# DoubangoTelecom/compv

Hardware: AMD Instinct MI355X
Metric: Mpixels/s Sobel->Canny->HoughSHT on 4K uint8 (higher is better)
Workload: dtype u8; 1 GPU; batched 3840x2160 uint8 frames, Sobel3x3 -> Canny(59,119) -> HoughSHT(rho=1, theta=1deg, thr=100); 256 distinct frames resident per GPU as 8 batches of 32, a step processes one batch, steps rotate over the batches; frames_per_gpu=32, resident_batches=8, parallelism=frames sharded across 1 GPU(s), no data-path collective

## Files before the change

compv_amd/csrc/api.cpp:

```cpp
#include "api_internal.hpp"

namespace {
__attribute__((noinline, optnone)) float libmCosf(float x) { return cosf(x); }
__attribute__((noinline, optnone)) float libmSinf(float x) { return sinf(x); }

void gradientThresholds(float fLow, float fHigh, int* tLow, int* tHigh)
{
	const float l = fLow < 1.f ? 1.f : (fLow > 65535.f ? 65535.f : fLow);
	const float h = fHigh < 1.f ? 1.f : (fHigh > 65535.f ? 65535.f : fHigh);
	uint16_t lo = static_cast<uint16_t>(l), hi = static_cast<uint16_t>(h);
	lo = static_cast<uint16_t>(std::max<int>(1, lo));
	hi = static_cast<uint16_t>(std::max<int>(lo + 2, hi));
	*tLow = lo; *tHigh = hi;
}

void cannyCoverage(size_t W, int* simdEnd, int* cStart)
{
	const size_t maxCols = W - 1;
	size_t mpw = 1;
	if (maxCols >= 16) mpw = 16; else if (maxCols >= 8) mpw = 8;
	if (mpw == 1) { *simdEnd = 1; *cStart = 1; return; }
	size_t col = 1;
	while (col + (mpw - 1) < maxCols) col += mpw;
	*simdEnd = static_cast<int>(col);
	*cStart = static_cast<int>(maxCols & static_cast<size_t>(-static_cast<ptrdiff_t>(mpw - 1)));
}

const float kPiF = 3.1415926535897932384626433f;
float piOver180() { return kPiF / 180.f; }

void shtTables(float thetaDeg, size_t T, std::vector<int32_t>& sinQ, std::vector<int32_t>& cosQ)
{
	const float fTheta = thetaDeg * piOver180();
	const float fRho = 1.f;
	sinQ.resize(T); cosQ.resize(T);
	float tt = 0.f;
	for (size_t t = 0; t < T; ++t, tt += fTheta) {
		sinQ[t] = static_cast<int32_t>((libmSinf(tt) * fRho) * 65535.f);
		cosQ[t] = static_cast<int32_t>((libmCosf(tt) * fRho) * 65535.f);
	}
}

static size_t voteMaxWindow()
{
	const char* e = getenv("COMPVHIP_VOTE_MAX_WINDOW");
	const long n = e ? atol(e) : 0;
	return (n >= 64 && n <= kShtMaxWindow) ? static_cast<size_t>(n) : static_cast<size_t>(kShtMaxWindow);
}

static bool voteGridTables(size_t W, size_t H, const std::vector<int32_t>& sinQ, const std::vector<int32_t>& cosQ, int split, int& nx, int& ny, int& TW, int& TH, long long& worst,
                           std::vector<int32_t>* kt, std::vector<int32_t>* rowBase)
{
	const size_t T = sinQ.size();
	const long long barrier = static_cast<long long>(W + H);
	nx = 1; ny = 1;
	for (int k = 0; k < split; ++k) {
		const double tw = static_cast<double>(W) / nx, th = static_cast<double>(H) / ny;
		if (tw >= th) ++nx; else ++ny;
	}
	TW = static_cast<int>(alignUp((W + nx - 1) / nx, 32)); TH = static_cast<int>((H + ny - 1) / ny);
	nx = static_cast<int>((W + TW - 1) / TW);
	const int tiles = nx * ny;
	if (kt) { kt->assign(static_cast<size_t>(tiles) * T, 0); rowBase->assign(static_cast<size_t>(tiles) * T, 0); }
	worst = 0;
	for (int ty = 0; ty < ny; ++ty) for (int tx = 0; tx < nx; ++tx) {
		const long long x0 = static_cast<long long>(tx) * TW, y0 = static_cast<long long>(ty) * TH;
		const long long mx = TW - 1, my = TH - 1;
		for (size_t t = 0; t < T; ++t) {
			const long long c = cosQ[t], sn = sinQ[t];
			const long long C = x0 * c + y0 * sn;
			long long Chi = C / 65536; if (C - Chi * 65536 < 0) --Chi;
			const long long Clo = C - Chi * 65536;
			const long long corners[4] = { Clo, mx * c + Clo, my * sn + Clo, mx * c + my * sn + Clo };
			long long qmin = 0, qmax = 0;
			for (int k = 0; k < 4; ++k) {
				long long q = corners[k] / 65536; if (corners[k] - q * 65536 < 0) --q;
				if (k == 0 || q < qmin) qmin = q;
				if (k == 0 || q > qmax) qmax = q;
			}
			const long long base = barrier - Chi - qmax;
			const long long d = ((base % 16) + 16) % 16;
			worst = std::max(worst, qmax - qmin + 1 + d);
			if (kt) {
				(*kt)[(static_cast<size_t>(ty) * nx + tx) * T + t] = static_cast<int32_t>((qmax + d) * 65536 + 65535 - Clo);
				(*rowBase)[(static_cast<size_t>(ty) * nx + tx) * T + t] = static_cast<int32_t>(base - d);
			}
		}
	}
	return alignUp(static_cast<size_t>(worst), 16) <= voteMaxWindow() && TW <= 1280 &&
	       static_cast<long long>(TW - 1) * 65535 + static_cast<long long>(TH - 1) * 65535 < 0x7f000000LL;
}

bool planVoteTiles(size_t W, size_t H, size_t frames, const std::vector<int32_t>& sinQ, const std::vector<int32_t>& cosQ, ShtTileArgs& v, std::vector<int32_t>& kt,
                   std::vector<int32_t>& rowBase)
{
	const size_t T = sinQ.size();
	const int groups = static_cast<int>((T + 63) / 64);
	int first = -1;
	for (int split = 0; split < 512 && first < 0; ++split) {
		int nx, ny, TW, TH; long long worst;
		if (voteGridTables(W, H, sinQ, cosQ, split, nx, ny, TW, TH, worst, nullptr, nullptr)) first = split;
	}
	if (first < 0) return false;
	int best = first; double bestCost = 0.0;
	int nx0, ny0, TW0, TH0; long long worst0;
	(void)voteGridTables(W, H, sinQ, cosQ, first, nx0, ny0, TW0, TH0, worst0, nullptr, nullptr);
	const bool starved = static_cast<double>(frames) * nx0 * ny0 * groups < 64.0;
	for (int split = first; starved && split <= first + 4; ++split) {
		int nx, ny, TW, TH; long long worst;
		if (!voteGridTables(W, H, sinQ, cosQ, split, nx, ny, TW, TH, worst, nullptr, nullptr)) continue;
		const double rw = static_cast<double>(alignUp(static_cast<size_t>(worst), 16));
		const double wgs = static_cast<double>(frames) * nx * ny * groups;
		const double rounds = wgs <= 1024.0 ? std::ceil(wgs / 256.0) : wgs / 256.0;
		const double perWg = 67.0 * (static_cast<double>(TW) * TH) / (960.0 * 720.0) + 9.3 * rw / 1208.0;
		const double reduce = 36.0 * (static_cast<double>(frames) * nx * ny * rw) / (32.0 * 12.0 * 1208.0);
		const double cost = rounds * perWg + reduce;
		if (split == first || cost < bestCost * 0.97) { best = split; bestCost = cost; }
	}
	int nx, ny, TW, TH; long long worst;
	if (!voteGridTables(W, H, sinQ, cosQ, best, nx, ny, TW, TH, worst, &kt, &rowBase)) return false;
	v.nx = nx; v.ny = ny; v.TW = TW; v.TH = TH; v.tiles = nx * ny;
	v.Rw = static_cast<int>(alignUp(static_cast<size_t>(worst), 16)); v.rwPitch = v.Rw;
	v.groups = groups; v.Tpad = v.groups * 64;
	v.tileCap = static_cast<size_t>(TW) * TH;
	return true;
}

ShtArgs shtArgs(compvhip_plan* p, int threshold)
{
	ShtArgs a;
	a.ebits = p->ebits; a.edges = p->edges; a.edgeCounts = p->edgeCounts; a.acc = p->acc;
	a.sinQ = p->sinQ; a.cosQ = p->cosQ; a.lineKeys = p->keysA; a.lineVals = p->valsA; a.lineCounts = p->lineCounts;
	a.frameTotals = p->frameTotals; a.lineTotal = p->lineTotal; a.sortN = 0; a.outCounts = nullptr; a.stepFlags = nullptr; a.hostStep = nullptr;
	a.nmsRange = p->nmsRange; a.blockCounts = p->blockCounts; a.lineBlocks = p->lineBlocks; a.nmsFlags = p->nmsFlags; a.nmsRows = static_cast<int>(sht_nms_rows(static_cast<int>(p->R))); a.nmsGroups = sht_nms_groups(static_cast<int>(p->T));
	a.bitsFrameStride = p->bitsFrameStride; a.edgeCap = p->edgeCap; a.accFrameStride = p->accFrameStride; a.lineCap = p->lineCap;
	a.W = static_cast<int>(p->W); a.H = static_cast<int>(p->H); a.wb = p->wb;
	a.R = static_cast<int>(p->R); a.T = static_cast<int>(p->T); a.accPitch = p->accPitch; a.barrier = static_cast<int>(p->W + p->H);
	a.threshold = threshold;
	a.nmsLastCol = static_cast<int>((p->T - 1) & ~static_cast<size_t>(3));
	a.frames = static_cast<int>(p->frames);
	a.strengthBits = p->strengthBits;
	return a;
}

int ensurePreproc(compvhip_plan* p)
{
	compvhip_ctx* ctx = p->ctx;
	if (!p->hist) HIPCHK(ctx, dmalloc(ctx, &p->hist, static_cast<size_t>(256) * kOtsuMaxChunks * p->frames));
	if (!p->otsu) HIPCHK(ctx, dmalloc(ctx, &p->otsu, p->frames));
	return COMPVHIP_OK;
}

int enqueueCanny(compvhip_plan* p, const uint8_t* d_in, uint8_t* d_out, int tLow, int tHigh, int ksize, int thrMode, float fLow, float fHigh, hipStream_t st)
{
	compvhip_ctx* ctx = p->ctx;
	CannyArgs a;
	a.zero = nullptr; a.nZero = 0;
	a.in = d_in; a.out = d_out; a.ebits = p->ebits; a.ubits = p->ubits; a.thrDev = (thrMode != COMPVHIP_CANNY_THRESHOLD_COMPARE_TO_GRADIENT) ? p->thrDev : nullptr;
	a.inFrameStride = p->S * p->H; a.outFrameStride = p->S * p->H; a.bitsFrameStride = p->bitsFrameStride;
	a.W = static_cast<int>(p->W); a.H = static_cast<int>(p->H); a.S = static_cast<int>(p->S); a.So = static_cast<int>(p->S);
	a.wb = p->wb; a.tilesX = p->tilesX; a.tilesY = p->tilesY; a.tLow = tLow; a.tHigh = tHigh; a.ksize = ksize;
	cannyCoverage(p->W, &a.simdEnd, &a.cStart);
	const bool gap = !((a.simdEnd >= a.W - 1) || (a.cStart <= a.simdEnd));
	if (thrMode == COMPVHIP_CANNY_THRESHOLD_OTSU) {
		int rc = ensurePreproc(p);
		if (rc) return rc;
		Stamp s(p, st, "otsu_kernels");
		HIPCHK(ctx, launch_otsu(d_in, a.W, a.H, a.S, a.inFrameStride, static_cast<int>(p->frames), fLow, fHigh, p->hist, p->otsu, p->thrDev, st));
	}
	if (thrMode == COMPVHIP_CANNY_THRESHOLD_PERCENT_OF_MEAN) {
		Stamp s(p, st, "canny_mean_thresholds");
		HIPCHK(ctx, launch_mean_thresholds(d_in, a.W, a.H, a.S, a.inFrameStride, static_cast<int>(p->frames), fLow, fHigh, p->sums, p->thrDev, st));
	}
	a.zero = p->counters; a.nZero = static_cast<int>(p->nCounts + kMaxRounds);
	p->countersFresh = true;
	p->roundsUsed = 0;
	{
		Stamp s(p, st, "canny_tile_kernel");
		HIPCHK(ctx, launch_canny_tiles(a, static_cast<int>(p->frames), gap, st));
	}
	return COMPVHIP_OK;
}

int enqueueResolve(compvhip_plan* p, uint8_t* d_out, int rounds, hipStream_t st)
{
	compvhip_ctx* ctx = p->ctx;
	ResolveArgs r;
	r.ebits = p->ebits; r.ubits = p->ubits; r.out = d_out; r.flags = p->flags; r.dirty = p->dirty;
	r.outFrameStride = p->S * p->H; r.bitsFrameStride = p->bitsFrameStride;
	r.H = static_cast<int>(p->H); r.So = static_cast<int>(p->S); r.wb = p->wb;
	for (int i = 0; i < rounds; ++i) {
		if (p->roundsUsed >= p->maxRounds) {
			HIPCHK(ctx, hipMemsetAsync(p->flags + 3, 0, sizeof(int) * (p->maxRounds - 3), st));
			HIPCHK(ctx, hipMemsetD32Async(reinterpret_cast<hipDeviceptr_t>(p->flags + 3), 1, 1, st));
			p->roundsUsed = 4;
		}
		r.round = p->roundsUsed++;
		Stamp s(p, st, "canny_resolve_kernel");
		HIPCHK(ctx, launch_canny_resolve(r, static_cast<int>(p->frames), st));
	}
	return COMPVHIP_OK;
}

int resolveConverged(compvhip_plan* p, hipStream_t st, bool* done)
{
	compvhip_ctx* ctx = p->ctx;
	const int last = p->roundsUsed - 1;
// ... 219 lines not shown
}

int compvhip_houghkht_to_cartesian(size_t W, size_t H, const compvhip_line* lines, size_t n, float* out)
{
	if (!W || !H || (n && (!lines || !out))) return COMPVHIP_E_INVALID_PARAMETER;
	const float widthF = static_cast<float>(W), heightF = static_cast<float>(H);
	const float r = std::sqrt((widthF * widthF) + (heightF * heightF));
	const float halfW = widthF * 0.5f, halfH = heightF * 0.5f;
	for (size_t i = 0; i < n; ++i, out += 4) {
		const float rho = lines[i].rho, theta = lines[i].theta;
		if (theta == 0.f) { out[0] = rho + halfW; out[1] = r; out[2] = rho + halfW; out[3] = -r; continue; }
		const float c = libmCosf(theta) * halfW, inv = 1.f / libmSinf(theta);
		out[0] = 0.f; out[1] = ((rho + c) * inv) + halfH;
		out[2] = widthF; out[3] = ((rho - c) * inv) + halfH;
	}
	return COMPVHIP_OK;
}

int compvhip_houghsht_vote_grid(size_t W, size_t H, float thetaDeg, size_t frames, int* nx, int* ny, int* windowRows)
{
	size_t R = 0, T = 0; float st = 0.f;
	if (!nx || !ny || !windowRows || !frames) return COMPVHIP_E_INVALID_PARAMETER;
	const int rc = shtDims(W, H, thetaDeg, &R, &T, &st);
	if (rc) return rc;
	if (T < 5) return COMPVHIP_E_NOT_IMPLEMENTED;
	std::vector<int32_t> sq, cq, kt, rb;
	shtTables(thetaDeg, T, sq, cq);
	ShtTileArgs v = {};
	if (!planVoteTiles(W, H, frames, sq, cq, v, kt, rb)) return COMPVHIP_E_NOT_IMPLEMENTED;
	*nx = v.nx; *ny = v.ny; *windowRows = v.Rw;
	return COMPVHIP_OK;
}

int compvhip_host_cpu_budget(void)
{
	return static_cast<int>(std::min<size_t>(hostCpuBudget(), 0x7fffffff));
}

int compvhip_houghsht_dims(size_t W, size_t H, float thetaDeg, size_t* R, size_t* T, float* step)
{
	if (!R || !T) return COMPVHIP_E_INVALID_PARAMETER;
	return shtDims(W, H, thetaDeg, R, T, step);
}

int compvhip_houghkht_dims(size_t W, size_t H, float rho, float thetaDeg, size_t* rhoN, size_t* T)
{
	KhtAxes ax;
	if (!rhoN || !T || !khtAxes(W, H, rho, thetaDeg, ax)) return COMPVHIP_E_INVALID_PARAMETER;
	*rhoN = ax.rhoN; *T = ax.T;
	return COMPVHIP_OK;
}

int compvhip_plan_create(compvhip_ctx* ctx, size_t W, size_t H, size_t S, size_t frames, float thetaDeg, compvhip_plan** out)
{
	if (!ctx || !out) return COMPVHIP_E_INVALID_PARAMETER;
	*out = nullptr;
	if (W < 3 || H < 3 || W > 32767 || H > 32767 || S < W || (S & 7) || !frames || !(thetaDeg > 0.f))
		return fail(ctx, COMPVHIP_E_INVALID_PARAMETER, "plan geometry (need 3 <= W,H <= 32767, S >= W, S % 8 == 0, frames > 0)");
	HIPCHK(ctx, hipSetDevice(ctx->device));
	compvhip_plan* p = new (std::nothrow) compvhip_plan();
	if (!p) return fail(ctx, COMPVHIP_E_OUT_OF_MEMORY, "plan");
	p->ctx = ctx; p->W = W; p->H = H; p->S = S; p->frames = frames; p->thetaDeg = thetaDeg;
	p->tilesX = static_cast<int>((W + 511) / 512);
	p->tilesY = static_cast<int>((H + 63) / 64);
	p->wb = p->tilesX * 16;
	p->bitsFrameStride = static_cast<size_t>(p->wb) * H;
	int rc = COMPVHIP_OK;
	do {
		if (dmalloc(ctx, &p->ebits, p->bitsFrameStride * frames) != hipSuccess) { rc = COMPVHIP_E_OUT_OF_MEMORY; break; }
		if (dmalloc(ctx, &p->ubits, p->bitsFrameStride * frames) != hipSuccess) { rc = COMPVHIP_E_OUT_OF_MEMORY; break; }
		if (hipMemset(p->ebits, 0, sizeof(uint32_t) * p->bitsFrameStride * frames) != hipSuccess) { rc = COMPVHIP_E_HIP; break; }
		if (hipMemset(p->ubits, 0, sizeof(uint32_t) * p->bitsFrameStride * frames) != hipSuccess) { rc = COMPVHIP_E_HIP; break; }
		if (hipDeviceSynchronize() != hipSuccess) { rc = COMPVHIP_E_HIP; break; }
		{
			p->voteTiles = true;
			size_t R = 0, T = 0; float step = 0.f;
			if (p->voteTiles && shtDims(W, H, thetaDeg, &R, &T, &step) == COMPVHIP_OK && T >= 5) {
				std::vector<int32_t> sq, cq;
				shtTables(thetaDeg, T, sq, cq);
				if (!planVoteTiles(W, H, frames, sq, cq, p->vt, p->vtKt, p->vtRowBase)) p->voteTiles = false;
			}
			else p->voteTiles = false;
			p->lineBlocks = p->voteTiles ? sht_lines_blocks(static_cast<int>(R)) : 0;
			p->nCounts = (2 + static_cast<size_t>(p->voteTiles ? p->vt.tiles : 0) + static_cast<size_t>(p->lineBlocks)) * frames + (frames + 1) * kFrameSlot;
		}
		if (dmalloc(ctx, &p->counters, p->nCounts + kMaxRounds) != hipSuccess) { rc = COMPVHIP_E_OUT_OF_MEMORY; break; }
		p->edgeCounts = p->counters; p->lineCounts = p->counters + frames; p->tileCounts = p->counters + 2 * frames; p->blockCounts = p->counters + (2 + static_cast<size_t>(p->voteTiles ? p->vt.tiles : 0)) * frames; p->flags = p->counters + p->nCounts;
		p->frameTotals = p->blockCounts + static_cast<size_t>(p->lineBlocks) * frames; p->lineTotal = reinterpret_cast<unsigned int*>(p->frameTotals + frames * kFrameSlot);
		if (const char* e = getenv("COMPVHIP_RESOLVE_WRAP")) { const int v = atoi(e); if (v >= 8 && v <= kMaxRounds && (v & 3) == 0) p->maxRounds = v; }
		if (hipMemset(p->counters, 0, sizeof(int) * (p->nCounts + kMaxRounds)) != hipSuccess) { rc = COMPVHIP_E_HIP; break; }
		if (dmalloc(ctx, &p->thrDev, frames) != hipSuccess) { rc = COMPVHIP_E_OUT_OF_MEMORY; break; }
		if (dmalloc(ctx, &p->dirty, canny_resolve_dirty_bytes(static_cast<int>(H), p->wb, static_cast<int>(frames))) != hipSuccess) { rc = COMPVHIP_E_OUT_OF_MEMORY; break; }
		if (dmalloc(ctx, &p->sums, frames * kFrameSlot) != hipSuccess) { rc = COMPVHIP_E_OUT_OF_MEMORY; break; }
		if (hipHostMalloc(reinterpret_cast<void**>(&p->hFlags), sizeof(int) * 2 * (kAsyncDepth + 1)) != hipSuccess) { rc = COMPVHIP_E_OUT_OF_MEMORY; break; }
		p->hTotals = reinterpret_cast<unsigned int*>(p->hFlags + kAsyncDepth + 1);
		if (hipHostMalloc(reinterpret_cast<void**>(&p->hRounds), sizeof(int) * (kFrameSlot + 4) * kAsyncDepth, hipHostMallocMapped) != hipSuccess) { rc = COMPVHIP_E_OUT_OF_MEMORY; break; }
		if (hipHostGetDevicePointer(reinterpret_cast<void**>(&p->hRoundsDev), p->hRounds, 0) != hipSuccess) { rc = COMPVHIP_E_HIP; break; }
	} while (0);
	if (rc) { compvhip_plan_destroy(p); return fail(ctx, rc, "plan allocation"); }
	*out = p;
	return COMPVHIP_OK;
}

void compvhip_plan_destroy(compvhip_plan* p)
{
	if (!p) return;
	compvhip_ctx* ctx = p->ctx;
	(void)hipSetDevice(ctx->device);
	timelineClear(p);
	for (hipEvent_t e : p->eventPool) (void)hipEventDestroy(e);
	for (auto& stp : p->steps) if (stp.done) (void)hipEventDestroy(stp.done);
	dfree(ctx, p->dirty);
	dfree(ctx, p->ebits); dfree(ctx, p->ubits); dfree(ctx, p->counters); dfree(ctx, p->thrDev); dfree(ctx, p->sums); dfree(ctx, p->tmpOut);
	if (p->hFlags) (void)hipHostFree(p->hFlags);
	if (p->hRounds) (void)hipHostFree(p->hRounds);
	dfree(ctx, p->hist); dfree(ctx, p->otsu); dfree(ctx, p->blurTmp); dfree(ctx, p->grayTmp);
	dfree(ctx, p->morphTmp);
	dfree(ctx, p->fastWork); dfree(ctx, p->fastScores);
	p->orbIndex.release(ctx); dfree(ctx, p->orbBlur);
	for (KhtBatchState* b : p->khtBatch) khtBatchFree(ctx, b);
	p->khtBatch.clear();
	dfree(ctx, p->cosT); dfree(ctx, p->invSinT);
	dfree(ctx, p->dKt); dfree(ctx, p->dRowBase); dfree(ctx, p->partLo); dfree(ctx, p->partHi); dfree(ctx, p->colFlag);
	dfree(ctx, p->sinQ); dfree(ctx, p->cosQ); dfree(ctx, p->edges); dfree(ctx, p->acc);
	dfree(ctx, p->keysA); dfree(ctx, p->keysB); dfree(ctx, p->valsA); dfree(ctx, p->valsB); dfree(ctx, p->nmsFlags); dfree(ctx, p->chunkHist); dfree(ctx, p->strengthStart);
	dfree(ctx, p->nmsRange); dfree(ctx, p->reach); dfree(ctx, p->sortTemp); p->segPerLine.release(ctx);
	dfree(ctx, p->compRows); dfree(ctx, p->compBits); dfree(ctx, p->compParent);
	delete p;
}

int compvhip_plan_set_timing(compvhip_plan* p, int enabled)
{
	if (!p) return COMPVHIP_E_INVALID_PARAMETER;
	p->timing = (enabled >= 2 && enabled <= 4) ? enabled : (enabled != 0 ? 1 : 0);
	return COMPVHIP_OK;
}

int compvhip_plan_get_timing(compvhip_plan* p, const char** names, float* ms, int cap)
{
	if (!p) return COMPVHIP_E_INVALID_PARAMETER;
	(void)hipSetDevice(p->ctx->device);
	if (!p->timeline.empty()) {
		for (auto& t : p->timeline) (void)hipEventSynchronize(t.b);
		timelineCollect(p);
	}
	const int n = std::min<int>(cap, static_cast<int>(p->timingMs.size()));
	for (int i = 0; i < n; ++i) { if (names) names[i] = p->timingNames[i].c_str(); if (ms) ms[i] = p->timingMs[i]; }
	return n;
}

static int planCannyImpl(compvhip_plan* p, const uint8_t* d_in, float tLow, float tHigh, int ksize, int type, uint8_t* d_edges, hipStream_t st,
                         bool waitConverged, bool clearTimeline = true)
{
	compvhip_ctx* ctx = p->ctx;
	if (!d_in || !d_edges) return fail(ctx, COMPVHIP_E_INVALID_PARAMETER, "null frame pointer");
	int lo, hi;
	int rc = validateCannyParams(ctx, tLow, tHigh, ksize, type, &lo, &hi);
	if (rc) return rc;
	HIPCHK(ctx, hipSetDevice(ctx->device));
	if (p->timing && clearTimeline) timelineClear(p);
	uint8_t* out = d_edges;
	const size_t bytes = p->S * p->H * p->frames;
	const bool alias = (d_in < d_edges + bytes) && (d_edges < d_in + bytes);
	if (alias) {
		if (!p->tmpOut) HIPCHK(ctx, dmalloc(ctx, &p->tmpOut, bytes));
		out = p->tmpOut;
	}
	p->patchOut = out;
	p->copyBack = alias ? d_edges : nullptr;
	if (p->W < static_cast<size_t>(ksize) || p->H < static_cast<size_t>(ksize)) return fail(ctx, COMPVHIP_E_INVALID_PARAMETER, "image smaller than the kernel");
// ... 424 lines not shown
```

compv_amd/csrc/api_internal.hpp:

```cpp
#pragma once
#include "../../include/compv_hip.h"
#include "kernels.hpp"
#include "kht.hpp"

#include <hip/hip_runtime.h>

#include <algorithm>
#include <atomic>
#include <chrono>
#include <cmath>
#include <cstdio>
#include <cstdlib>
#include <cstring>
#include <functional>
#include <memory>
#include <string>
#include <thread>
#include <vector>

using namespace compvhip;

namespace compvhip_api {
void countLive(compvhip_ctx* ctx, long delta);

// ... 72 lines not shown
};

struct KhtBatchFrame {
	KhtBitPlane plane; size_t most = 0, ptsOff = 0, nPts = 0;
	std::vector<KhtRange> strings; size_t slotBase = 0, slots = 0;
	uint32_t nClusters = 0;
	std::vector<KhtKernel> kernels; double hmax = 0.0, GS = 1.0; bool haveGS = false;
	std::vector<KhtVoteParams> params; size_t paramsBase = 0;
	std::vector<KhtCell> cells; size_t cellOff = 0; int cellCount = 0;
	KhtPeaksWork peaks; std::vector<KhtLine> out;
	double ms[6] = {};
	int code = COMPVHIP_OK; std::string err;
};
struct KhtBatchState {
	hipStream_t stream = nullptr;
	DevBuf<uint32_t> dBits; PinBuf<uint32_t> hostBits;
	std::vector<hipEvent_t> ready;
	PinBuf<KhtPoint> linked; DevBuf<KhtPoint> pts;
	DevBuf<KhtStringDesc> strings; DevBuf<uint32_t> counts32; PinBuf<KhtStringDesc> stringsHost;
	DevBuf<uint32_t> totals;
	DevBuf<KhtSpan> spans, scratch; DevBuf<KhtSubdivFrame> stack; DevBuf<KhtKernel> kernelsDev;
	PinBuf<KhtKernel> kernelsHost;
	DevBuf<int32_t> counts;
	DevBuf<KhtVoteParams> params; PinBuf<KhtVoteParams> paramsHost;
	DevBuf<KhtCell> cells; DevBuf<int> cellCount; PinBuf<KhtCell> cellsHost;
	KhtCanonTabs tabs; DevBuf<KhtLine> canonLines; DevBuf<int32_t> canonCounts;
	PinBuf<KhtLine> canonLinesHost;
	std::vector<KhtBatchFrame> frames;
	hipEvent_t syncEv = nullptr;
	double stageMs[6] = {};
};

struct compvhip_ctx {
	int device = 0;
	std::string err;
	std::atomic<long> live{0};
	hipStream_t stream = nullptr;
	compvhip_plan* hostPlan = nullptr;
	DevBuf<uint8_t> dIn, dOut;
	DevBuf<uint8_t> dPacked;
	DevBuf<uint32_t> dHist;
	DevBuf<int32_t> dCounts, dAccOut;
	DevBuf<compvhip_line> dSegLines;
	DevBuf<compvhip_segment> dSegs;
	DevBuf<int32_t> dSegCount;
	DevBuf<compvhip_line_fit> dFits;
	DevBuf<int32_t> dFitCount;
	DevBuf<compvhip_line> dFitRefined;
	DevBuf<int32_t> dCompLabels;
	DevBuf<compvhip_component> dComps;
	DevBuf<int32_t> dCompCount;
	DevBuf<compvhip_corner> dFastCorners;
	DevBuf<int32_t> dFastCount;
	DevBuf<compvhip_keypoint> dOrbKeys;
	DevBuf<int32_t> dOrbCount;
	DevBuf<uint8_t> dOrbDesc;
	KhtScratch kht;
};

struct TimingEntry { const char* name; hipEvent_t a, b; };
struct TimingState {
	int timing = 0;
	std::vector<hipEvent_t> eventPool;
	std::vector<TimingEntry> timeline;
	std::vector<std::string> timingNames; std::vector<float> timingMs;
};

struct StepParams {
	const uint8_t* d_in = nullptr; float tLow = 0.f, tHigh = 0.f; int threshold = 0, maxLines = 0;
	int ksize = 3, thresholdType = COMPVHIP_CANNY_THRESHOLD_COMPARE_TO_GRADIENT, pixfmt = COMPVHIP_FMT_Y;
	uint8_t* d_gray = nullptr; int32_t* d_otsu = nullptr; float* d_cart = nullptr;
	uint8_t* d_edges = nullptr; compvhip_line* d_lines = nullptr; size_t lineCap = 0; int32_t* d_counts = nullptr;
};

struct compvhip_plan : TimingState {
	compvhip_ctx* ctx = nullptr;
	size_t W = 0, H = 0, S = 0, frames = 0;
	float thetaDeg = 1.f;
	int tilesX = 0, tilesY = 0, wb = 0;
	size_t bitsFrameStride = 0;
	uint32_t* ebits = nullptr; uint32_t* ubits = nullptr;
	int* counters = nullptr;
	size_t nCounts = 0;
	int* flags = nullptr; int* hFlags = nullptr;
	int* frameTotals = nullptr; unsigned int* lineTotal = nullptr;
	unsigned int* hTotals = nullptr;
	unsigned int recentTotals[8] = {}; int recentN = 0;
	int specRounds = kSpecRounds; unsigned char recentRounds[8] = {}; int recentRoundsN = 0;
	int* hRoundsDev = nullptr; int* stepHostSlot = nullptr;
	int* hRounds = nullptr;
	int roundsUsed = 0;
	int maxRounds = kMaxRounds;
	bool countersFresh = false;
	int2* thrDev = nullptr; unsigned int* sums = nullptr;
	uint8_t* dirty = nullptr;
	uint8_t* patchOut = nullptr; uint8_t* copyBack = nullptr;
	uint8_t* grayTmp = nullptr;
	uint8_t* tmpOut = nullptr;
	bool bitsValid = false;
	bool shtReady = false;
	size_t R = 0, T = 0; float thetaStep = 0.f; int accPitch = 0;
	uint8_t* blurTmp = nullptr;
	uint32_t* hist = nullptr; int32_t* otsu = nullptr;
	float* cosT = nullptr; float* invSinT = nullptr;
	int32_t* sinQ = nullptr; int32_t* cosQ = nullptr;
	uint32_t* edges = nullptr; size_t edgeCap = 0; int* edgeCounts = nullptr;
	uint16_t* acc = nullptr; size_t accFrameStride = 0;
	uint32_t* keysA = nullptr; uint32_t* keysB = nullptr; uint32_t* valsA = nullptr; uint32_t* valsB = nullptr; size_t lineCap = 0; int* lineCounts = nullptr;
	int2* reach = nullptr;
	int2* nmsRange = nullptr;
	uint8_t* nmsFlags = nullptr;
	int* blockCounts = nullptr; int lineBlocks = 0;
	void* sortTemp = nullptr; size_t sortTempBytes = 0;
	DevBuf<int32_t> segPerLine;
	int32_t* compRows = nullptr; uint32_t* compBits = nullptr; int32_t* compParent = nullptr;
	uint8_t* morphTmp = nullptr;
	int* fastWork = nullptr; uint8_t* fastScores = nullptr;
	DevBuf<int32_t> orbIndex; uint8_t* orbBlur = nullptr; uint16_t orbKern[5] = {}; bool orbKernReady = false; bool orbBriefLds = false;
	int strengthBits = 16, keyBits = 0;
	uint16_t* chunkHist = nullptr; uint32_t* strengthStart = nullptr; int sortChunks = 0; bool deviceSort = false;
	bool voteTiles = false;
	ShtTileArgs vt = {};
	std::vector<int32_t> vtKt, vtRowBase;
	int32_t* dKt = nullptr; int32_t* dRowBase = nullptr; uint8_t* partLo = nullptr; uint8_t* partHi = nullptr; uint8_t* colFlag = nullptr; int* tileCounts = nullptr;
	std::vector<KhtBatchState*> khtBatch;
	std::vector<std::unique_ptr<KhtPeaksWork>> khtWork;
	double khtStageMs[6] = {}; double khtWallMs = 0.0; int khtThreads = 0;
	struct AsyncStep { bool used = false; bool replay = false; uint64_t seq = 0; hipEvent_t done = nullptr; hipStream_t stream = nullptr; StepParams sp; size_t sortN = 0; int rounds = 0; } steps[kAsyncDepth];
	uint64_t stepSeq = 0;
};

struct compvhip_matcher : TimingState {
	compvhip_ctx* ctx = nullptr;
	int descDwords = 0, queryCap = 0, trainCap = 0, pairs = 0, knn = 0;
	uint32_t* partial = nullptr;
	compvhip_match* reverse = nullptr;
};
namespace compvhip_api {

inline void countLive(compvhip_ctx* ctx, long delta) { ctx->live += delta; }

inline int fail(compvhip_ctx* ctx, int code, const char* what, hipError_t e = hipSuccess)
{
	if (ctx) {
		ctx->err = what ? what : "";
		if (e != hipSuccess) { ctx->err += ": "; ctx->err += hipGetErrorString(e); }
	}
	return code;
}

#define HIPCHK(ctx, call) do { hipError_t e__ = (call); if (e__ != hipSuccess) return fail((ctx), COMPVHIP_E_HIP, #call, e__); } while (0)

inline size_t alignUp(size_t v, size_t a) { return (v + a - 1) / a * a; }

inline bool stampWanted(const compvhip_plan* p, const char* name)
{
	if (p->timing == 1) return true;
	if (p->timing == 2) return !strcmp(name, "canny_tile_kernel") || !strcmp(name, "sht_vote_kernel");
	if (p->timing == 3) return !strcmp(name, "sht_vote_kernel");
	if (p->timing == 4) return !strcmp(name, "canny_tile_kernel");
	return false;
}

inline bool takeEvent(TimingState* p, hipEvent_t* e)
{
	if (!p->eventPool.empty()) { *e = p->eventPool.back(); p->eventPool.pop_back(); return true; }
// ... 66 lines not shown
```

compv_amd/csrc/kernels.hpp:

```cpp
#pragma once
#include <hip/hip_runtime.h>
#include <stddef.h>
#include <stdint.h>

#include "../../include/compv_hip.h"

namespace compvhip {

#ifndef COMPVHIP_BAND_H
#define COMPVHIP_BAND_H 64
#endif
constexpr int kBandH = COMPVHIP_BAND_H;
#ifndef COMPVHIP_BAND_WORDS
#define COMPVHIP_BAND_WORDS 64
#endif
constexpr int kBandWords = COMPVHIP_BAND_WORDS;
constexpr int kResolveThreads = 512;
constexpr int kFrameSlot = 32;
constexpr int kResolveRows = kBandH * kBandWords / kResolveThreads;

struct CannyArgs {
	const uint8_t* in;
	uint8_t* out;
	uint32_t* ebits;
// ... 30 lines not shown

struct EdgeDeteArgs {
	const uint8_t* in;
	uint8_t* out;
	unsigned int* gmax;
	size_t inFrameStride, outFrameStride;
	int W, H, S, So;
	int tilesX, tilesY;
	int blockRows, groups;
};
hipError_t launch_edge_dete(const EdgeDeteArgs& a, int op, int frames, hipStream_t stream);

struct GrayArgs {
	const uint8_t* in;
	uint8_t* out;
	int W, H, S, So;
};
hipError_t launch_gray(const GrayArgs& a, int fmt, int frames, hipStream_t stream);
constexpr int kOtsuMaxChunks = 128;
hipError_t launch_otsu(const uint8_t* in, int W, int H, int S, size_t frameStride, int frames, float fLowFactor, float fHighFactor, uint32_t* hist,
                       int32_t* otsu, void* thr, hipStream_t stream);

constexpr int kFxpMaxTaps = 15;
struct FxpArgs {
	const uint8_t* in;
	uint8_t* out;
	size_t inFrameStride, outFrameStride;
	int W, H, S, So;
	uint32_t kern[kFxpMaxTaps];
};
hipError_t launch_convlt_fxp(const uint8_t* in, uint8_t* tmp, uint8_t* out, int W, int H, int S, size_t frameStride, int frames, const uint16_t* vtKern,
                             const uint16_t* hzKern, int K, hipStream_t stream);

struct I16Args {
	const void* in;
	int16_t* out;
	int W, H, S, So, K;
	int kern[kFxpMaxTaps];
};
hipError_t launch_convlt_i16(const void* in, bool inIsU8, int16_t* tmp, int16_t* out, int W, int H, int S, int So, const int16_t* vtKern, const int16_t* hzKern,
                             int K, hipStream_t stream);

struct ShtArgs {
	const uint32_t* ebits;
	uint32_t* edges;
	int* edgeCounts;
	uint16_t* acc;
	const int32_t* sinQ;
	const int32_t* cosQ;
	uint32_t* lineKeys;
	uint32_t* lineVals;
	uint8_t* nmsFlags;
	int nmsRows;
	int* blockCounts;
	int lineBlocks;
	const int2* nmsRange;
	int nmsGroups;
	int* lineCounts;
	const int* stepFlags;
	int* hostStep;
	int32_t* outCounts;
	int* frameTotals;
	unsigned int* lineTotal;
	size_t sortN;
	size_t bitsFrameStride, edgeCap, accFrameStride, lineCap;
	int W, H, wb;
	int R, T, accPitch, barrier;
	int threshold, nmsLastCol;
	int frames;
	int strengthBits;
};
struct ShtTileArgs {
	const int32_t* kt;
	const int32_t* rowBase;
	uint8_t* partLo;
	uint8_t* partHi;
	uint8_t* colFlag;
	const int2* reach;
	int* tileCounts;
	int nx, ny, TW, TH, tiles;
	int Rw, rwPitch;
	int Tpad, groups;
	size_t tileCap;
};
constexpr int kShtMaxWindow = 1264;
hipError_t launch_sht_compact_tiles(const ShtArgs& a, const ShtTileArgs& v, int frames, hipStream_t stream);
hipError_t launch_sht_vote_tiles(const ShtArgs& a, const ShtTileArgs& v, int frames, hipStream_t stream);
hipError_t launch_sht_reduce_tiles(const ShtArgs& a, const ShtTileArgs& v, int frames, hipStream_t stream);
hipError_t launch_bytes_to_bits(const uint8_t* edges, int W, int H, int S, size_t frameStride, uint32_t* ebits, int wb, size_t bitsFrameStride,
                                int frames, hipStream_t stream);
hipError_t launch_sht_lines(const ShtArgs& a, int frames, hipStream_t stream);
hipError_t launch_sht_decode(const uint32_t* keys, const uint32_t* vals, const int* counts, size_t lineCap, int frames, int T, int barrier, float thetaStep,
                             int maxLines, int strengthBits, void* lines , size_t outCap, hipStream_t stream);
int sht_nms_groups(int T);
size_t sht_nms_rows(int R);
int sht_lines_blocks(int R);
hipError_t launch_sht_cartesian(const void* lines , const int* counts, size_t lineCap, int maxLines, int frames, int T, const float* cosT,
                                const float* invSinT, float thetaStep, float widthF, float r, float* out , hipStream_t stream);
hipError_t launch_sht_acc_transpose(const uint16_t* accT, int R, int T, int accPitch, int32_t* out, size_t outStride, hipStream_t stream);
constexpr int kShtSortChunk = 4096;
constexpr int kShtSortMaxStrengthBits = 13;
constexpr int kShtSortMaxChunks = 32;
struct ShtSortArgs {
	uint32_t* sortedKeys;
	uint32_t* sortedVals;
	uint16_t* chunkHist;
	uint32_t* strengthStart;
	int chunks;
};
hipError_t launch_sht_sort_lines(const ShtArgs& a, const ShtSortArgs& q, int frames, float thetaStep, int maxLines, void* lines , size_t outCap,
                                 hipStream_t stream);
hipError_t sht_sort_pairs(void* temp, size_t& tempBytes, const uint32_t* keysIn, uint32_t* keysOut, const uint32_t* valsIn, uint32_t* valsOut, size_t n,
                          int keyBits, hipStream_t stream);

struct ShtLineSetArgs {
	const uint32_t* ebits;
	const uint8_t* edges;
	size_t bitsFrameStride, edgeFrameStride;
	int wb, S;
	const int32_t* sinQ;
	const int32_t* cosQ;
	const compvhip_line* lines;
	const int32_t* lineCounts;
	size_t lineCap;
	int nLines;
	int W, H, R, T, barrier;
};
struct ShtSegArgs : ShtLineSetArgs {
	int minLength, maxGap;
	int32_t* perLine;
	compvhip_segment* segs;
	size_t segCap;
	int32_t* segCounts;
	int frame0;
};
hipError_t launch_sht_segments(const ShtSegArgs& a, int frames, int phase, hipStream_t stream);

struct ShtFitArgs : ShtLineSetArgs {
	int halfWidth;
	const compvhip_segment* segs;
	const int32_t* segCounts;
	size_t segCap;
	compvhip_line_fit* fits;
	size_t fitCap;
	int32_t* fitCounts;
	compvhip_line* refined;
	int frame0;
};
static_assert(sizeof(ShtLineSetArgs) == 104 && sizeof(ShtSegArgs) == 152 && sizeof(ShtFitArgs) == 176, "kernel argument layout");
hipError_t launch_sht_fit(const ShtFitArgs& a, int frames, hipStream_t stream);

struct CompArgs {
	const uint32_t* bits;
	size_t bitsFrameStride;
	int wb;
	int W, H;
	int words;
	uint32_t lastMask;
	int conn8;
	int minPixels;
	int32_t* parent;
	size_t parentFrameStride;
	int ps;
	int wantLabels;
	compvhip_component* comps;
	size_t compCap;
// ... 116 lines not shown
```

compv_amd/csrc/sht_tiles_kernels.hip:

```cpp
#include "device.hpp"

namespace compvhip {

constexpr int kTcThreads = 256;
constexpr int kTcRows = 64;
constexpr int kTcStage = 6144;

__global__ __launch_bounds__(kTcThreads) void sht_compact_tiles_kernel(ShtArgs a, ShtTileArgs v)
{
	__shared__ int s_wave[kTcThreads / 64];
	__shared__ int s_base;
	__shared__ uint32_t s_stage[kTcStage];
	const int frame = blockIdx.y;
	const int chunksPerTile = (v.TH + kTcRows - 1) / kTcRows;
	const int tile = blockIdx.x / chunksPerTile, chunk = blockIdx.x - tile * chunksPerTile;
	const int ty = tile / v.nx, tx = tile - ty * v.nx;
	const int x0 = tx * v.TW, y0 = ty * v.TH;
	const int wpr = v.TW >> 5;
	const uint32_t wprInv = (1u << 20) / (uint32_t)wpr + 1u;
	const int ly0 = chunk * kTcRows;
	const int rows = min(min(kTcRows, v.TH - ly0), a.H - (y0 + ly0));
	const int nwords = max(rows, 0) * wpr;
	const uint32_t* __restrict__ bits = a.ebits + (size_t)frame * a.bitsFrameStride;
	const int w0 = x0 >> 5;
	constexpr int kPer = (kTcRows * 40 + kTcThreads - 1) / kTcThreads;
	uint32_t wv[kPer]; int wl[kPer];
	int cnt = 0;
	if (nwords == 0) return;
#pragma unroll
	for (int k = 0; k < kPer; ++k) {
		const int i = min((int)threadIdx.x + k * kTcThreads, nwords - 1);
		const int r = (int)(((uint32_t)i * wprInv) >> 20), c = i - r * wpr;
		wv[k] = bits[(size_t)(y0 + ly0 + r) * a.wb + min(w0 + c, a.wb - 1)];
		wl[k] = ((ly0 + r) << 16) | (c << 5);
	}
#pragma unroll
	for (int k = 0; k < kPer; ++k) {
		const int i = (int)threadIdx.x + k * kTcThreads;
		const int c = (wl[k] & 0xffff) >> 5;
		if (!(i < nwords && w0 + c < a.wb)) wv[k] = 0u;
		cnt += __popc(wv[k]);
	}
	const int lane = threadIdx.x & 63, wave = threadIdx.x >> 6;
	const int incl = wave_incl_scan(cnt, lane);
	if (lane == 63) s_wave[wave] = incl;
	__syncthreads();
	int wbase = 0, total = 0;
#pragma unroll
	for (int k = 0; k < kTcThreads / 64; ++k) {
		const int t = s_wave[k];
		if (k < wave) wbase += t;
		total += t;
	}
	if (total == 0) return;
	if (threadIdx.x == 0) s_base = atomicAdd(&v.tileCounts[frame * v.tiles + tile], total);
	__syncthreads();
	uint32_t* __restrict__ dst = a.edges + ((size_t)frame * v.tiles + tile) * v.tileCap;
	const int first = wbase + (incl - cnt);
	if (total <= kTcStage) {
		int lp = first;
#pragma unroll
		for (int k = 0; k < kPer; ++k) {
			uint32_t b = wv[k];
			while (b) {
				const int bit = __ffs(b) - 1;
				b &= b - 1;
				s_stage[lp++] = (uint32_t)(wl[k] + bit);
			}
		}
		__syncthreads();
		const size_t room = (size_t)s_base < v.tileCap ? v.tileCap - (size_t)s_base : 0;
		const int nout = (int)min((size_t)total, room);
		for (int i = threadIdx.x; i < nout; i += kTcThreads) dst[(size_t)s_base + i] = s_stage[i];
		return;
	}
	size_t pos = (size_t)s_base + first;
#pragma unroll
	for (int k = 0; k < kPer; ++k) {
		uint32_t b = wv[k];
		while (b) {
			const int bit = __ffs(b) - 1;
			b &= b - 1;
			if (pos < v.tileCap) dst[pos] = (uint32_t)(wl[k] + bit);
			++pos;
		}
	}
}

constexpr int kVtThreads = 1024;
constexpr int kVtUnroll = 32;

__global__ __launch_bounds__(kVtThreads) void sht_vote_tiles_kernel(ShtArgs a, ShtTileArgs v)
{
	extern __shared__ __attribute__((aligned(16))) uint32_t hist[];
	const int units = a.frames * v.tiles;
	const int xcd = blockIdx.x & 7, k = blockIdx.x >> 3;
	const int g = k % v.groups;
	const int unit = (k / v.groups) * 8 + xcd;
	if (unit >= units) return;
	const int frame = unit / v.tiles, tile = unit - frame * v.tiles;
	const int tid = threadIdx.x, lane = tid & 63;
	const int wave = __builtin_amdgcn_readfirstlane(tid >> 6);

	const int nAll = v.tileCounts[unit];
	if (g == 0 && threadIdx.x == 0 && nAll) atomicAdd(&a.edgeCounts[frame], nAll);
	const int n = min(nAll, (int)v.tileCap);
	const int words = v.Rw * 32;
	uint32_t* const s_any = hist + words;
	if (tid < 2) s_any[tid] = 0u;
	for (int i = tid * 4; i < words; i += kVtThreads * 4) *reinterpret_cast<uint4*>(&hist[i]) = make_uint4(0, 0, 0, 0);

	const int t = g * 64 + lane;
	const int tt = min(t, a.T - 1);
	const int nc = -a.cosQ[tt], ns = -a.sinQ[tt];
	const int K = v.kt[(size_t)tile * a.T + tt];
	uint32_t inc = (t < a.T) ? ((lane & 32) ? 0x10000u : 1u) : 0u;
	asm volatile("" : "+v"(inc));
	const uint32_t lane4 = (uint32_t)(lane & 31) * 4u;
	__syncthreads();

	const uint32_t* __restrict__ list = a.edges + (size_t)unit * v.tileCap;
	typedef uint32_t u32x16 __attribute__((ext_vector_type(16)));
	auto vote = [&](uint32_t e) {
		const int lx = (int)(e & 0xffffu), ly = (int)(e >> 16);
		int val, ad;
		asm volatile("v_mad_i32_i24 %0, %1, %2, %3" : "=v"(val) : "s"(lx), "v"(nc), "v"(K));
		asm volatile("v_mad_i32_i24 %0, %1, %2, %3" : "=v"(val) : "s"(ly), "v"(ns), "v"(val));
		const uint32_t row = (uint32_t)val >> 16;
		asm volatile("v_lshl_add_u32 %0, %1, 7, %2" : "=v"(ad) : "v"(row), "v"(lane4));
		asm volatile("ds_add_u32 %0, %1" : : "v"(ad), "v"(inc) : "memory");
	};
	const int nblk = n / kVtUnroll;
	constexpr int kStep = kVtThreads / 64;
	u32x16 a0, a1, b0, b1;
#define VT_LOAD(r0, r1, blk) asm volatile("s_load_dwordx16 %0, %2, 0x0\n\ts_load_dwordx16 %1, %2, 0x40" : "=&s"(r0), "=&s"(r1) : "s"(list + (size_t)(blk) * kVtUnroll) : "memory")
#define VT_WAIT(r0, r1) asm volatile("s_waitcnt lgkmcnt(0)" : "+s"(r0), "+s"(r1) : : "memory")
#define VT_VOTE(r0, r1) _Pragma("unroll") for (int u = 0; u < 16; ++u) vote(r0[u]); _Pragma("unroll") for (int u = 0; u < 16; ++u) vote(r1[u])
	int b = wave;
	if (b < nblk) {
		VT_LOAD(a0, a1, b);
		VT_WAIT(a0, a1);
		for (;;) {
			const int bn = b + kStep;
			if (bn < nblk) VT_LOAD(b0, b1, bn);
			VT_VOTE(a0, a1);
			if (bn >= nblk) break;
			VT_WAIT(b0, b1);
			b = bn + kStep;
			if (b < nblk) VT_LOAD(a0, a1, b);
			VT_VOTE(b0, b1);
			if (b >= nblk) break;
			VT_WAIT(a0, a1);
		}
	}
#undef VT_LOAD
#undef VT_WAIT
#undef VT_VOTE
	for (int i = nblk * kVtUnroll + wave; i < n; i += kStep) vote(__builtin_amdgcn_readfirstlane(list[i]));
	__builtin_amdgcn_s_waitcnt(0xc07f);
	__syncthreads();

	const size_t column = ((size_t)unit * v.Tpad) + (size_t)g * 64 + lane;
	uint8_t* __restrict__ partLo = v.partLo + column * v.rwPitch;
	uint8_t* __restrict__ partHi = v.partHi + column * v.rwPitch;
	const uint32_t sel1 = (lane & 32) ? 0x07030602u : 0x05010400u;
	typedef uint32_t u32x4 __attribute__((ext_vector_type(4)));
	auto bytes16 = [&](int w0, u32x4& lo, u32x4& hi) {
		uint32_t h[16];
#pragma unroll
		for (int j = 0; j < 16; ++j) h[j] = hist[(w0 + j) * 32 + (lane & 31)];
#pragma unroll
		for (int q = 0; q < 4; ++q) {
			const uint32_t p01 = __builtin_amdgcn_perm(h[4 * q + 1], h[4 * q], sel1), p23 = __builtin_amdgcn_perm(h[4 * q + 3], h[4 * q + 2], sel1);
			lo[q] = __builtin_amdgcn_perm(p23, p01, 0x05040100u);
			hi[q] = __builtin_amdgcn_perm(p23, p01, 0x07060302u);
		}
	};
	uint32_t any = 0u;
	for (int wb = wave * 128; wb < v.Rw; wb += (kVtThreads / 64) * 128)
	for (int w0 = wb; w0 < min(wb + 128, v.Rw); w0 += 16) {
		u32x4 lo, hi;
		bytes16(w0, lo, hi);
		any |= hi.x | hi.y | hi.z | hi.w;
		uint8_t* const dst = partLo + w0;
		asm volatile("global_store_dwordx4 %0, %1, off" : : "v"(dst), "v"(lo) : "memory");
	}
	const uint64_t mine = __ballot(any != 0u);
	if (lane == 0 && mine) { atomicOr(&s_any[0], (uint32_t)mine); atomicOr(&s_any[1], (uint32_t)(mine >> 32)); }
	__syncthreads();
	const uint32_t m0 = s_any[0], m1 = s_any[1];
	const bool flagged = (((lane & 32) ? m1 : m0) >> (lane & 31)) & 1u;
	if (wave == 0) v.colFlag[column] = flagged ? 1 : 0;
	if ((m0 | m1) == 0u) return;
	if (flagged) {
		for (int wb = wave * 128; wb < v.Rw; wb += (kVtThreads / 64) * 128)
		for (int w0 = wb; w0 < min(wb + 128, v.Rw); w0 += 16) {
			u32x4 lo, hi;
			bytes16(w0, lo, hi);
			uint8_t* const dst = partHi + w0;
			asm volatile("global_store_dwordx4 %0, %1, off" : : "v"(dst), "v"(hi) : "memory");
		}
	}
}

constexpr int kRdThreads = 64;
constexpr int kRdRows = 16;

__global__ __launch_bounds__(kRdThreads) void sht_reduce_tiles_kernel(ShtArgs a, ShtTileArgs v)
{
	const int frame = blockIdx.z, theta = blockIdx.y;
	const int2 reach = v.reach[theta];
	if ((int)(blockIdx.x * kRdThreads * kRdRows) >= reach.y || (int)((blockIdx.x + 1) * kRdThreads * kRdRows) <= reach.x) return;
	const int r0 = (blockIdx.x * kRdThreads + threadIdx.x) * kRdRows;
	if (r0 >= a.accPitch) return;
	uint32_t E[4] = { 0, 0, 0, 0 }, O[4] = { 0, 0, 0, 0 };
	int covers = 0;
	for (int tile = 0; tile < v.tiles; ++tile) {
		const int base = v.rowBase[(size_t)tile * a.T + theta];
		const int w0 = r0 - base;
		if (w0 < 0 || w0 >= v.Rw) continue;
		++covers;
		const size_t column = ((size_t)frame * v.tiles + tile) * v.Tpad + theta;
		const uint4 c = *reinterpret_cast<const uint4*>(v.partLo + column * v.rwPitch + w0);
		E[0] += c.x & 0x00ff00ffu; O[0] += (c.x >> 8) & 0x00ff00ffu;
		E[1] += c.y & 0x00ff00ffu; O[1] += (c.y >> 8) & 0x00ff00ffu;
		E[2] += c.z & 0x00ff00ffu; O[2] += (c.z >> 8) & 0x00ff00ffu;
		E[3] += c.w & 0x00ff00ffu; O[3] += (c.w >> 8) & 0x00ff00ffu;
		if (v.colFlag[column]) {
			const uint4 h = *reinterpret_cast<const uint4*>(v.partHi + column * v.rwPitch + w0);
			E[0] += (h.x & 0x00ff00ffu) << 8; O[0] += h.x & 0xff00ff00u;
			E[1] += (h.y & 0x00ff00ffu) << 8; O[1] += h.y & 0xff00ff00u;
			E[2] += (h.z & 0x00ff00ffu) << 8; O[2] += h.z & 0xff00ff00u;
			E[3] += (h.w & 0x00ff00ffu) << 8; O[3] += h.w & 0xff00ff00u;
		}
	}
	if (!covers) return;
	uint32_t o[8];
#pragma unroll
	for (int d = 0; d < 4; ++d) {
		o[2 * d] = (E[d] & 0xffffu) | (O[d] << 16);
		o[2 * d + 1] = (E[d] >> 16) | (O[d] & 0xffff0000u);
// ... 44 lines not shown
```

Baseline: 426,700 Mpixels/s.

## Split per-tile edge lists into 256-row bands with packed 8-bit row offsets

Edge lists for each vote tile are now stored per 256-row band, each band with its own counter. Entries encode the local row in the top 8 bits instead of 16. The vote kernel walks the bands through a lane-held table and folds each band's y-offset into a per-block constant, so it can take the x term straight from the scalar word without masking. It also adds a per-band remainder pass and a TH<=1280 limit, which means extra counters, band-lookup logic and atomics spread over more addresses.

```diff
diff --git a/compv_amd/csrc/api.cpp b/compv_amd/csrc/api.cpp
--- a/compv_amd/csrc/api.cpp
+++ b/compv_amd/csrc/api.cpp
@@ -87,7 +87,7 @@
 			}
 		}
 	}
-	return alignUp(static_cast<size_t>(worst), 16) <= voteMaxWindow() && TW <= 1280 &&
+	return alignUp(static_cast<size_t>(worst), 16) <= voteMaxWindow() && TW <= 1280 && TH <= 1280 &&
 	       static_cast<long long>(TW - 1) * 65535 + static_cast<long long>(TH - 1) * 65535 < 0x7f000000LL;
 }
 
@@ -123,6 +123,7 @@
 	v.Rw = static_cast<int>(alignUp(static_cast<size_t>(worst), 16)); v.rwPitch = v.Rw;
 	v.groups = groups; v.Tpad = v.groups * 64;
 	v.tileCap = static_cast<size_t>(TW) * TH;
+	v.bands = (TH + 255) / 256;
 	return true;
 }
 
@@ -508,10 +509,11 @@
 			}
 			else p->voteTiles = false;
 			p->lineBlocks = p->voteTiles ? sht_lines_blocks(static_cast<int>(R)) : 0;
-			p->nCounts = (2 + static_cast<size_t>(p->voteTiles ? p->vt.tiles : 0) + static_cast<size_t>(p->lineBlocks)) * frames + (frames + 1) * kFrameSlot;
+			p->nTileCounts = p->voteTiles ? static_cast<size_t>(p->vt.tiles) * p->vt.bands : 0;
+		p->nCounts = (2 + p->nTileCounts + static_cast<size_t>(p->lineBlocks)) * frames + (frames + 1) * kFrameSlot;
 		}
 		if (dmalloc(ctx, &p->counters, p->nCounts + kMaxRounds) != hipSuccess) { rc = COMPVHIP_E_OUT_OF_MEMORY; break; }
-		p->edgeCounts = p->counters; p->lineCounts = p->counters + frames; p->tileCounts = p->counters + 2 * frames; p->blockCounts = p->counters + (2 + static_cast<size_t>(p->voteTiles ? p->vt.tiles : 0)) * frames; p->flags = p->counters + p->nCounts;
+		p->edgeCounts = p->counters; p->lineCounts = p->counters + frames; p->tileCounts = p->counters + 2 * frames; p->blockCounts = p->counters + (2 + p->nTileCounts) * frames; p->flags = p->counters + p->nCounts;
 		p->frameTotals = p->blockCounts + static_cast<size_t>(p->lineBlocks) * frames; p->lineTotal = reinterpret_cast<unsigned int*>(p->frameTotals + frames * kFrameSlot);
 		if (const char* e = getenv("COMPVHIP_RESOLVE_WRAP")) { const int v = atoi(e); if (v >= 8 && v <= kMaxRounds && (v & 3) == 0) p->maxRounds = v; }
 		if (hipMemset(p->counters, 0, sizeof(int) * (p->nCounts + kMaxRounds)) != hipSuccess) { rc = COMPVHIP_E_HIP; break; }
diff --git a/compv_amd/csrc/api_internal.hpp b/compv_amd/csrc/api_internal.hpp
--- a/compv_amd/csrc/api_internal.hpp
+++ b/compv_amd/csrc/api_internal.hpp
@@ -178,6 +178,7 @@
 	uint32_t* ebits = nullptr; uint32_t* ubits = nullptr;
 	int* counters = nullptr;
 	size_t nCounts = 0;
+	size_t nTileCounts = 0;
 	int* flags = nullptr; int* hFlags = nullptr;
 	int* frameTotals = nullptr; unsigned int* lineTotal = nullptr;
 	unsigned int* hTotals = nullptr;
diff --git a/compv_amd/csrc/kernels.hpp b/compv_amd/csrc/kernels.hpp
--- a/compv_amd/csrc/kernels.hpp
+++ b/compv_amd/csrc/kernels.hpp
@@ -136,6 +136,7 @@
 	int Rw, rwPitch;
 	int Tpad, groups;
 	size_t tileCap;
+	int bands;
 };
 constexpr int kShtMaxWindow = 1264;
 hipError_t launch_sht_compact_tiles(const ShtArgs& a, const ShtTileArgs& v, int frames, hipStream_t stream);
diff --git a/compv_amd/csrc/sht_tiles_kernels.hip b/compv_amd/csrc/sht_tiles_kernels.hip
--- a/compv_amd/csrc/sht_tiles_kernels.hip
+++ b/compv_amd/csrc/sht_tiles_kernels.hip
@@ -4,6 +4,8 @@
 
 constexpr int kTcThreads = 256;
 constexpr int kTcRows = 64;
+constexpr int kBandRows = 256;
+constexpr int kMaxBands = 5;
 constexpr int kTcStage = 6144;
 
 __global__ __launch_bounds__(kTcThreads) void sht_compact_tiles_kernel(ShtArgs a, ShtTileArgs v)
@@ -24,7 +26,7 @@
 	const uint32_t* __restrict__ bits = a.ebits + (size_t)frame * a.bitsFrameStride;
 	const int w0 = x0 >> 5;
 	constexpr int kPer = (kTcRows * 40 + kTcThreads - 1) / kTcThreads;
-	uint32_t wv[kPer]; int wl[kPer];
+	uint32_t wv[kPer], wl[kPer];
 	int cnt = 0;
 	if (nwords == 0) return;
 #pragma unroll
@@ -32,12 +34,12 @@
 		const int i = min((int)threadIdx.x + k * kTcThreads, nwords - 1);
 		const int r = (int)(((uint32_t)i * wprInv) >> 20), c = i - r * wpr;
 		wv[k] = bits[(size_t)(y0 + ly0 + r) * a.wb + min(w0 + c, a.wb - 1)];
-		wl[k] = ((ly0 + r) << 16) | (c << 5);
+		wl[k] = ((uint32_t)((ly0 & (kBandRows - 1)) + r) << 24) | (uint32_t)(c << 5);
 	}
 #pragma unroll
 	for (int k = 0; k < kPer; ++k) {
 		const int i = (int)threadIdx.x + k * kTcThreads;
-		const int c = (wl[k] & 0xffff) >> 5;
+		const int c = (int)(wl[k] & 0xffffu) >> 5;
 		if (!(i < nwords && w0 + c < a.wb)) wv[k] = 0u;
 		cnt += __popc(wv[k]);
 	}
@@ -53,9 +55,11 @@
 		total += t;
 	}
 	if (total == 0) return;
-	if (threadIdx.x == 0) s_base = atomicAdd(&v.tileCounts[frame * v.tiles + tile], total);
-	__syncthreads();
-	uint32_t* __restrict__ dst = a.edges + ((size_t)frame * v.tiles + tile) * v.tileCap;
+	const int band = ly0 / kBandRows;
+	const size_t bandCap = (size_t)min(kBandRows, v.TH - band * kBandRows) * v.TW;
+	if (threadIdx.x == 0) s_base = atomicAdd(&v.tileCounts[((size_t)frame * v.tiles + tile) * v.bands + band], total);
+	__syncthreads();
+	uint32_t* __restrict__ dst = a.edges + ((size_t)frame * v.tiles + tile) * v.tileCap + (size_t)band * kBandRows * v.TW;
 	const int first = wbase + (incl - cnt);
 	if (total <= kTcStage) {
 		int lp = first;
@@ -65,11 +69,11 @@
 			while (b) {
 				const int bit = __ffs(b) - 1;
 				b &= b - 1;
-				s_stage[lp++] = (uint32_t)(wl[k] + bit);
+				s_stage[lp++] = wl[k] + (uint32_t)bit;
 			}
 		}
 		__syncthreads();
-		const size_t room = (size_t)s_base < v.tileCap ? v.tileCap - (size_t)s_base : 0;
+		const size_t room = (size_t)s_base < bandCap ? bandCap - (size_t)s_base : 0;
 		const int nout = (int)min((size_t)total, room);
 		for (int i = threadIdx.x; i < nout; i += kTcThreads) dst[(size_t)s_base + i] = s_stage[i];
 		return;
@@ -81,7 +85,7 @@
 		while (b) {
 			const int bit = __ffs(b) - 1;
 			b &= b - 1;
-			if (pos < v.tileCap) dst[pos] = (uint32_t)(wl[k] + bit);
+			if (pos < bandCap) dst[pos] = wl[k] + (uint32_t)bit;
 			++pos;
 		}
 	}
@@ -102,9 +106,17 @@
 	const int tid = threadIdx.x, lane = tid & 63;
 	const int wave = __builtin_amdgcn_readfirstlane(tid >> 6);
 
-	const int nAll = v.tileCounts[unit];
+	const int* __restrict__ counts = v.tileCounts + (size_t)unit * v.bands;
+	int cnt[kMaxBands], nAll = 0;
+#pragma unroll
+	for (int k = 0; k < kMaxBands; ++k) cnt[k] = __builtin_amdgcn_readfirstlane(counts[min(k, v.bands - 1)]);
+#pragma unroll
+	for (int k = 0; k < kMaxBands; ++k) {
+		if (k >= v.bands) cnt[k] = 0;
+		nAll += cnt[k];
+		cnt[k] = min(cnt[k], max(min(kBandRows, v.TH - k * kBandRows), 0) * v.TW);
+	}
 	if (g == 0 && threadIdx.x == 0 && nAll) atomicAdd(&a.edgeCounts[frame], nAll);
-	const int n = min(nAll, (int)v.tileCap);
 	const int words = v.Rw * 32;
 	uint32_t* const s_any = hist + words;
 	if (tid < 2) s_any[tid] = 0u;
@@ -120,35 +132,62 @@
 	__syncthreads();
 
 	const uint32_t* __restrict__ list = a.edges + (size_t)unit * v.tileCap;
+	const int bandStride = kBandRows * v.TW;
 	typedef uint32_t u32x16 __attribute__((ext_vector_type(16)));
-	auto vote = [&](uint32_t e) {
-		const int lx = (int)(e & 0xffffu), ly = (int)(e >> 16);
+	auto bandK = [&](int y) {
+		int kb;
+		asm volatile("v_mad_i32_i24 %0, %1, %2, %3" : "=v"(kb) : "s"(y), "v"(ns), "v"(K));
+		return kb;
+	};
+	auto vote = [&](uint32_t e, int kb) {
+		const int lyr = (int)(e >> 24);
 		int val, ad;
-		asm volatile("v_mad_i32_i24 %0, %1, %2, %3" : "=v"(val) : "s"(lx), "v"(nc), "v"(K));
-		asm volatile("v_mad_i32_i24 %0, %1, %2, %3" : "=v"(val) : "s"(ly), "v"(ns), "v"(val));
+		asm volatile("v_mad_i32_i24 %0, %1, %2, %3" : "=v"(val) : "s"(e), "v"(nc), "v"(kb));
+		asm volatile("v_mad_i32_i24 %0, %1, %2, %3" : "=v"(val) : "s"(lyr), "v"(ns), "v"(val));
 		const uint32_t row = (uint32_t)val >> 16;
 		asm volatile("v_lshl_add_u32 %0, %1, 7, %2" : "=v"(ad) : "v"(row), "v"(lane4));
 		asm volatile("ds_add_u32 %0, %1" : : "v"(ad), "v"(inc) : "memory");
 	};
-	const int nblk = n / kVtUnroll;
+	int tab = 0, nblk = 0;
+#pragma unroll
+	for (int k = 0; k < kMaxBands; ++k) {
+		tab = (lane == k) ? nblk : tab;
+		tab = (lane == 8 + k) ? k * bandStride - nblk * kVtUnroll : tab;
+		tab = (lane == 16 + k) ? cnt[k] : tab;
+		nblk += cnt[k] / kVtUnroll;
+	}
+	tab = (lane == kMaxBands) ? nblk : tab;
 	constexpr int kStep = kVtThreads / 64;
+	int bandEnd = 0, adj = 0, bandY = 0;
+	auto locate = [&](int f) {
+		if (f < bandEnd) return;
+		int k = 0;
+#pragma unroll
+		for (int j = 1; j < kMaxBands; ++j) k = (f >= __builtin_amdgcn_readlane(tab, j)) ? j : k;
+		bandY = k * kBandRows;
+		adj = __builtin_amdgcn_readlane(tab, 8 + k);
+		bandEnd = __builtin_amdgcn_readlane(tab, 1 + k);
+	};
 	u32x16 a0, a1, b0, b1;
-#define VT_LOAD(r0, r1, blk) asm volatile("s_load_dwordx16 %0, %2, 0x0\n\ts_load_dwordx16 %1, %2, 0x40" : "=&s"(r0), "=&s"(r1) : "s"(list + (size_t)(blk) * kVtUnroll) : "memory")
+	int ka = K, kb = K;
+#define VT_LOAD(r0, r1, kr, blk) do { locate(blk); \
+		asm volatile("s_load_dwordx16 %0, %2, 0x0\n\ts_load_dwordx16 %1, %2, 0x40" : "=&s"(r0), "=&s"(r1) : "s"(list + ((size_t)(blk) * kVtUnroll + adj)) : "memory"); \
+		kr = bandK(bandY); } while (0)
 #define VT_WAIT(r0, r1) asm volatile("s_waitcnt lgkmcnt(0)" : "+s"(r0), "+s"(r1) : : "memory")
-#define VT_VOTE(r0, r1) _Pragma("unroll") for (int u = 0; u < 16; ++u) vote(r0[u]); _Pragma("unroll") for (int u = 0; u < 16; ++u) vote(r1[u])
+#define VT_VOTE(r0, r1, kr) _Pragma("unroll") for (int u = 0; u < 16; ++u) vote(r0[u], kr); _Pragma("unroll") for (int u = 0; u < 16; ++u) vote(r1[u], kr)
 	int b = wave;
 	if (b < nblk) {
-		VT_LOAD(a0, a1, b);
+		VT_LOAD(a0, a1, ka, b);
 		VT_WAIT(a0, a1);
 		for (;;) {
 			const int bn = b + kStep;
-			if (bn < nblk) VT_LOAD(b0, b1, bn);
-			VT_VOTE(a0, a1);
+			if (bn < nblk) VT_LOAD(b0, b1, kb, bn);
+			VT_VOTE(a0, a1, ka);
 			if (bn >= nblk) break;
 			VT_WAIT(b0, b1);
 			b = bn + kStep;
-			if (b < nblk) VT_LOAD(a0, a1, b);
-			VT_VOTE(b0, b1);
+			if (b < nblk) VT_LOAD(a0, a1, ka, b);
+			VT_VOTE(b0, b1, kb);
 			if (b >= nblk) break;
 			VT_WAIT(a0, a1);
 		}
@@ -156,7 +195,27 @@
 #undef VT_LOAD
 #undef VT_WAIT
 #undef VT_VOTE
-	for (int i = nblk * kVtUnroll + wave; i < n; i += kStep) vote(__builtin_amdgcn_readfirstlane(list[i]));
+	constexpr int kRemPer = (kVtUnroll - 1 + kStep - 1) / kStep;
+	uint32_t re[kMaxBands * kRemPer];
+#pragma unroll
+	for (int k = 0; k < kMaxBands; ++k) {
+		const int c = __builtin_amdgcn_readlane(tab, 16 + k), rem = c % kVtUnroll, at = k * bandStride + (c - rem);
+#pragma unroll
+		for (int j = 0; j < kRemPer; ++j) {
+			const int i = wave + j * kStep;
+			re[k * kRemPer + j] = __builtin_amdgcn_readfirstlane(list[i < rem ? at + i : 0]);
+		}
+	}
+#pragma unroll
+	for (int k = 0; k < kMaxBands; ++k) {
+		const int rem = __builtin_amdgcn_readlane(tab, 16 + k) % kVtUnroll;
+		if (wave < rem) {
+			const int kr = bandK(k * kBandRows);
+#pragma unroll
+			for (int j = 0; j < kRemPer; ++j)
+				if (wave + j * kStep < rem) vote(re[k * kRemPer + j], kr);
+		}
+	}
 	__builtin_amdgcn_s_waitcnt(0xc07f);
 	__syncthreads();
 
```

New measurement: 420,100 Mpixels/s. -1.5%, worse.
